# Jiahao-Ma/VFA

Hardware: AMD Instinct MI355X
Metric: voxels aggregated/sec (7 views->BEV grid) (higher is better)
Workload: dtype f32; 1 GPU; multiviewc_200x200x1; cameras_per_rank=7, cameras_total=7, channels=256, rccl_ranks=1, parallelism=single GPU

## Files before the change

include/vfa_hip.h:

```cpp
#ifndef VFA_HIP_H
#define VFA_HIP_H

#include <stddef.h>
#include <stdint.h>

#ifdef __cplusplus
extern "C" {
#endif

#define VFA_ABI_VERSION 9

#define VFA_CONV_MULTIVIEWC 0
#define VFA_CONV_MULTIVIEWX 1
#define VFA_CONV_WILDTRACK 2

#define VFA_VOX_REFERENCE 0
#define VFA_VOX_LAYER_MAJOR 1

#define VFA_VOX_KERNEL_DIRECT 0x100
#define VFA_VOX_KERNEL_TAP_CACHE 0x200

#define VFA_ERR_BAD_ARGUMENT 10001
#define VFA_ERR_UNSUPPORTED 10002

int vfa_abi_version(void);

#define VFA_FLAG_TERMS_MASK 0xf
#define VFA_FLAG_RESERVED_CUS(n) (((n) & 0xff) << 8)
#define VFA_FLAG_DEBUG(mask) (((mask) & 0xfff) << 16)
#define VFA_FLAG_DUMP_VOX (1 << 30)
#define VFA_FLAG_ROWS_ONLY (1 << 28)
#define VFA_FLAG_SKIP_ROWS (1 << 29)
#define VFA_BWD_ACCUMULATE 1

int vfa_integral_image_f32(const float *feature, float *integral, int n_views, int C, int Hf, int Wf,
                           void *stream);

int vfa_affine_relu_integral_image_f32(const float *x, const float *scale, const float *shift, float *integral, int n_views, int C,
                                       int Hf, int Wf, void *stream);

size_t vfa_feature_stats_count(int n_views, int C, int Hf);
int vfa_integral_images_f32(const float *const *features, const float *const *scales, const float *const *shifts,
                            float *const *integrals, unsigned *const *absmax, int n_views, int C, int n_maps, const int *feat_hw,
                            void *stream);
int vfa_integral_absmax_f32(const float *integral, unsigned *absmax, int n_views, int C, int Hf, int Wf, void *stream);

int vfa_integral_images_hwc_f32(const float *const *features_hwc, const float *const *scales, const float *const *shifts,
                                float *const *integrals, unsigned *const *absmax, int n_views, int C, int n_maps, const int *feat_hw,
                                void *stream);

size_t vfa_lateral_conv_workspace_bytes(int n_views, int Hf, int Wf);
int vfa_lateral_conv_f32(const float *feat, const float *weight, const float *bias, const float *gamma, const float *beta, float eps,
                         float *out_hwc, float *scale, float *shift, void *workspace, size_t workspace_bytes, int n_views, int K,
                         int Hf, int Wf, void *stream);
int vfa_lateral_convs_f32(int n_maps, const float *const *feats, const float *const *weights, const float *const *biases,
                          const float *const *gammas, const float *const *betas, const float *eps, float *const *outs_hwc,
                          float *const *scales, float *const *shifts, void *const *workspaces, const size_t *workspace_bytes, int n_views,
                          const int *Ks, const int *feat_hw, void *stream);

int vfa_lateral_convs_train_f32(int n_maps, const float *const *feats, const float *const *weights, const float *const *biases,
                                const float *const *gammas, const float *const *betas, const float *eps, float *const *outs_hwc,
                                float *const *scales, float *const *shifts, double *const *means, double *const *rstds,
// ... 210 lines not shown
```

vfa_amd/_lib.py:

```python
import ctypes
import os

_HERE = os.path.dirname(os.path.abspath(__file__))
LIB_PATH = os.environ.get("VFA_AMD_LIB") or os.path.join(_HERE, "csrc", "libvfa_hip.so")
ABI_VERSION = 9

CONV_KIND = {"MultiviewC": 0, "MultiviewX": 1, "Wildtrack": 2}
VOX_REFERENCE, VOX_LAYER_MAJOR = 0, 1
VOX_KERNEL_DIRECT, VOX_KERNEL_TAP_CACHE = 0x100, 0x200
BWD_ACCUMULATE = 1


FLAG_ROWS_ONLY, FLAG_SKIP_ROWS = 1 << 28, 1 << 29
FLAG_DUMP_VOX = 1 << 30


def collapse_flags(terms=0, reserved_cus=0):
    return (int(terms) & 0xf) | ((int(reserved_cus) & 0xff) << 8)


_c_int, _c_float, _c_size_t, _vp, _c_longlong = ctypes.c_int, ctypes.c_float, ctypes.c_size_t, ctypes.c_void_p, ctypes.c_longlong
_c_double = ctypes.c_double

SIGNATURES = {
    "vfa_abi_version": [],
    "vfa_integral_image_f32": [_vp, _vp, _c_int, _c_int, _c_int, _c_int, _vp],
    "vfa_affine_relu_integral_image_f32": [_vp, _vp, _vp, _vp, _c_int, _c_int, _c_int, _c_int, _vp],
    "vfa_box_params_f32": [_vp, _vp, _vp, _vp, _c_int, _c_int, _c_int, _c_int, _c_float, _c_float, _c_int, _c_int,
                           _c_float, _c_float, _vp, _vp, _vp, _vp],
    "vfa_gather_f32": [_vp, _vp, _vp, _vp, _vp, _c_int, _c_int, _c_int, _c_int, _c_int, _c_int, _c_int, _c_int, _c_int,
                       _vp],
    "vfa_project_gather_f32": [_vp, _vp, _vp, _vp, _vp, _vp, _c_int, _c_int, _c_int, _c_int, _c_int, _c_int, _c_int,
                               _c_int, _c_int, _c_float, _c_float, _c_float, _c_float, _c_int, _vp],
    "vfa_project_collapse_f32": [_vp, _vp, _vp, _vp, _vp, _vp, _vp, _c_int, _c_int, _c_int, _c_int, _c_int, _c_int, _c_int,
                                 _c_int, _c_float, _c_float, _c_float, _c_float, _vp],
    "vfa_gather_workspace_bytes": [_c_int, _c_int, _c_int],
    "vfa_project_gather_ws_f32": [_vp, _vp, _vp, _vp, _vp, _vp, _vp, _c_size_t, _c_int, _c_int, _c_int, _c_int, _c_int,
                                  _c_int, _c_int, _c_int, _c_int, _c_float, _c_float, _c_float, _c_float, _c_int, _vp],
    "vfa_project_gather_backward_f32": [_vp, _vp, _vp, _vp, _vp, _vp, _c_int, _c_int, _c_int, _c_int, _c_int, _c_int,
                                        _c_int, _c_int, _c_int, _c_float, _c_float, _c_float, _c_float, _c_int, _vp],
    "vfa_project_gather_backward_grid_f32": [_vp, _vp, _vp, _vp, _vp, _vp, _c_int, _c_int, _c_int, _c_int, _c_int, _c_int,
                                             _c_int, _c_int, _c_int, _c_int, _c_float, _c_float, _c_float, _c_float, _c_int, _vp],
    "vfa_gather_backward_det_workspace_bytes": [_c_int, _c_int, _c_int, _c_int, _c_int, _c_int],
    "vfa_project_gather_backward_det_f32": [_vp, _vp, _vp, _vp, _vp, _vp, _c_int, _c_int, _c_int, _c_int, _c_int, _c_int,
                                            _c_int, _c_int, _c_int, _c_int, _c_float, _c_float, _c_float, _c_float, _c_int, _vp,
                                            _c_size_t, _vp],
    "vfa_gather_backward_geometry_workspace_bytes": [_c_int, _c_int],
# ... 150 lines not shown
```

vfa_amd/csrc/vfa_fused.hip:

```cpp
#include <hip/hip_runtime.h>
#include <stdint.h>
#include <type_traits>

#include "vfa_geom.h"
#include "vfa_split.h"
#include "vfa_tile.h"

#ifndef VFA_TICKET_ORDER
#define VFA_TICKET_ORDER __ATOMIC_RELAXED
#endif

namespace {
using namespace vfa_dev;

constexpr int kRecBytes = 96;
constexpr int kMaxSlots = 123;
constexpr unsigned kItemCost = 704, kRowItemCost = 522;
constexpr int kRecSlots = 3;
constexpr int kThreads = 512;
constexpr int kRowBytes = 2 * kC;
constexpr int kPlane = kTileBoxes * kRowBytes;
constexpr int kSteps = kC / 16;

constexpr int kCont = 1 << 8;
constexpr int kTileRows = 4;
constexpr int kTileShiftAt = 8;

typedef int i32x8 __attribute__((ext_vector_type(8)));

struct RecordArgs {
    BoxGeom g;
    int n_views, L, W, tiles_w, n_tiles, n_scales;
    ScaleDims dims[kMaxScales];
    unsigned *live[kMaxScales];
    unsigned *direct[kMaxScales];
    unsigned *overflow[kMaxScales];
    unsigned *row_counter;
    unsigned rows_cap;
    unsigned *row_list;
    unsigned char *hdrs[kMaxScales];
    unsigned char *recs[kMaxScales];
    unsigned short *item_w;
    int views_pad;
};

__global__ __launch_bounds__(kWave) void frame_records_kernel(RecordArgs a)
{
    __shared__ uint4 stage[2][kTileBoxes * 6];
    const TileLane ln = tile_lane(a.n_views, a.n_tiles, a.tiles_w, a.L, a.W);
    const int lane = threadIdx.x, half = ln.half, b = ln.b, view = ln.view, tile = ln.tile;
    const bool pair_ok = ln.pair_ok, valid = ln.valid;

    float l, t, r, bt;
    cube_box(a.g, a.g.calibs + (size_t)view * 12, ln.cell, 0, l, t, r, bt);
#pragma unroll 1
    for (int s = 0; s < a.n_scales; ++s) {
        const int Hf = a.dims[s].Hf, Wf = a.dims[s].Wf;
        const float area = box_area(l, t, r, bt, Hf, Wf);
        const bool vis = valid && box_visible(area, Hf, Wf);
        const float masked = valid ? area * 0.0f : 0.0f;
        const bool live_box = vis || (valid && masked != masked);
        const BoxTaps tp = box_taps(l, t, r, bt, Hf, Wf);
        const int dx = tp.xr.i0 - tp.xl.i0, dy = tp.yb.i0 - tp.yt.i0;
        const int dxc = dx == 0 ? 0 : (dx == 1 ? 1 : 2), dyc = dy == 0 ? 0 : (dy == 1 ? 1 : 2);
        const TileWindow tw = tile_window(tp, vis, live_box, area, Hf, Wf, half);
        const Window &win = tw.w;
        const bool any_live = tw.any_live;
        const int shift = tw.shift, n_slots = win.n_slots;
        const bool direct = n_slots > kMaxSlots;
        unsigned rows[4], cols[4];
        tap_parts(win, tp, direct, rows, cols);
        const int tag = (vis ? 1 : 0) | (dxc << 1) | (dyc << 3);
        const unsigned kx = (unsigned)(tp.xs[0] + 1) | ((unsigned)(tp.xs[2] + 1) << 16), ky = (unsigned)(tp.ys[0] + 1) | ((unsigned)(tp.ys[2] + 1) << 16);
        const int tag_p = __shfl_up(tag, 1);
        const unsigned kx_p = __shfl_up(kx, 1), ky_p = __shfl_up(ky, 1);
        const bool cont = vis && (b & 3) != 0 && tag_p == tag && kx_p == kx && ky_p == ky;
// ... 6 lines not shown
            bilinear_weights(q, tp.xr, tp.yt); w[8] = q[0]; w[9] = q[1]; w[10] = q[2]; w[11] = q[3];
            bilinear_weights(q, tp.xl, tp.yb); w[12] = q[0]; w[13] = q[1]; w[14] = q[2]; w[15] = q[3];
        }
        if (pair_ok) {
            uint4 *st = stage[half] + b * 6;
            st[0] = make_uint4(__float_as_uint(w[0]), __float_as_uint(w[1]), __float_as_uint(w[2]), __float_as_uint(w[3]));
            st[1] = make_uint4(__float_as_uint(w[4]), __float_as_uint(w[5]), __float_as_uint(w[6]), __float_as_uint(w[7]));
            st[2] = make_uint4(__float_as_uint(w[8]), __float_as_uint(w[9]), __float_as_uint(w[10]), __float_as_uint(w[11]));
            st[3] = make_uint4(__float_as_uint(w[12]), __float_as_uint(w[13]), __float_as_uint(w[14]), __float_as_uint(w[15]));
            const float rcp = 1.0f / area;
            st[4] = make_uint4(__float_as_uint(rcp), (unsigned)tag | (cont ? (unsigned)kCont : 0u), rows[0] | (rows[1] << 16),
                               rows[2] | (rows[3] << 16));
            st[5] = make_uint4(cols[0] | (cols[1] << 16), cols[2] | (cols[3] << 16), __float_as_uint(masked), __float_as_uint(area));
        }
        __syncthreads();
        if (pair_ok) {
            uint4 *rec = reinterpret_cast<uint4 *>(a.recs[s] + ((size_t)view * a.n_tiles + tile) * kTileBoxes * kRecBytes);
#pragma unroll
            for (int k = 0; k < 6; ++k) rec[k * 32 + b] = stage[half][k * 32 + b];
            if (b == 0) {
                uint4 *hdr = reinterpret_cast<uint4 *>(a.hdrs[s] + ((size_t)view * a.n_tiles + tile) * kHdrBytes);
                unsigned hflags = (any_live ? kTileLive : 0) | (direct ? kTileDirect : 0) | ((unsigned)shift << kTileShiftAt), word2 = (unsigned)win.cwid;
                if (any_live) atomicOr(a.live[s] + tile, 1u << view);
                if (any_live && direct) {
                    atomicOr(a.direct[s] + tile, 1u << view);
                    const unsigned slot = atomicAdd(a.row_counter, 1u);
                    if (slot < a.rows_cap) {
                        hflags |= kTileRows; word2 = slot;
                        a.row_list[slot] = ((unsigned)s << 30) | ((unsigned)view << 25) | (unsigned)tile;
                    }
                    else atomicOr(a.overflow[s] + tile, 1u << view);
                }
                const bool main_item = any_live && !(direct && !(hflags & kTileRows));
                a.item_w[((size_t)tile * kMaxScales + s) * a.views_pad + view] =
                    (unsigned short)(!main_item ? 0u : (direct ? kRowItemCost : kItemCost + (unsigned)n_slots));
                hdr[0] = tile_header0(hflags, win, word2);
                hdr[1] = tile_header1(win);
            }
        }
        __syncthreads();
        if (blockIdx.x == 0 && lane < 6)
            reinterpret_cast<uint4 *>(a.recs[s] + (size_t)a.n_views * a.n_tiles * kTileBoxes * kRecBytes)[lane] = make_uint4(0u, 0u, 0u, 0u);
    }
}

struct ShiftArgs {
    BoxGeom g;
    int n_views, L, W, tiles_w, n_tiles, nl, Hf, Wf, per_item;
    unsigned char *out;
    unsigned *tile_max;
};
__global__ __launch_bounds__(kWave) void sliver_shift_kernel(ShiftArgs a)
{
    const TileLane ln = tile_lane(a.n_views, a.n_tiles, a.tiles_w, a.L, a.W);
    const float *P = a.g.calibs + (size_t)ln.view * 12;
    int shift = 0;
    for (int layer = 0; layer < a.nl; ++layer) {
        float l, t, r, bt;
        cube_box(a.g, P, ln.cell, layer, l, t, r, bt);
        const float area = box_area(l, t, r, bt, a.Hf, a.Wf);
        if (ln.valid && box_visible(area, a.Hf, a.Wf)) shift = max(shift, sliver_shift(area, a.Hf, a.Wf));
    }
#pragma unroll
    for (int m = 1; m < 32; m <<= 1) shift = max(shift, __shfl_xor(shift, m, 32));
    if (a.per_item) {
        if (ln.valid) a.out[(size_t)ln.view * a.L * a.W + ln.cell] = (unsigned char)shift;
    } else if (ln.pair_ok && ln.b == 0 && shift > 0) {
        atomicMax(a.tile_max + ln.tile, (unsigned)shift);
    }
}
__global__ __launch_bounds__(256) void sliver_expand_kernel(const unsigned *tile_max, unsigned char *out, int L, int W, int tiles_w)
{
    const int cell = blockIdx.x * 256 + threadIdx.x;
    if (cell >= L * W) return;
    const int cl = cell / W, cw = cell - cl * W;
    out[cell] = (unsigned char)tile_max[(cl / kTileL) * tiles_w + cw / kTileW];
}

constexpr int kWmaxParts = 32;
struct SplitArgs { const float *w[kMaxScales]; uint4 *out[kMaxScales]; unsigned *wmax; int *wexp; int f16; };
constexpr int kSplitBlocks = 8 * kSteps * 64 / 1024;
__device__ __forceinline__ void split_block(const SplitArgs &sa, int b, unsigned long long *part)
{
    const int scale = b / kSplitBlocks, j = b - scale * kSplitBlocks, tid = threadIdx.x;
    const float *__restrict__ w = sa.w[scale];
    uint4 *__restrict__ out = sa.out[scale];
    int ew = 0;
    if (sa.f16) {
        unsigned m = 0u;
        for (int i = tid; i < kC * kC; i += 1024) m = max(m, __float_as_uint(w[i]) & 0x7fffffffu);
        m = wave_max_u32(m);
        if ((tid & 63) == 0) part[tid >> 6] = m;
        __syncthreads();
        unsigned mm = 0u;
        for (int i = 0; i < 16; ++i) mm = max(mm, (unsigned)part[i]);
        ew = split_exponent(mm, kExpW);
    }
    const int idx = j * 1024 + tid;
    const int lane = idx & 63, st = (idx >> 6) & 15, wave = idx >> 10;
    const float *src = w + (size_t)(wave * 32 + (lane & 31)) * kC + 16 * st + 8 * (lane >> 5);
    if (idx == 0 && scale == 0) sa.wexp[kMaxScales] = sa.f16 ? 2 : 3;
    uint4 uh, ul;
    if (sa.f16) {
        fp16_saturate_mode(true);
        if (idx == 0) sa.wexp[scale] = ew;
        const float sc = pow2f(ew);
        uint2 h0, l0, h1, l1;
        split_f16x4(src[0] * sc, src[1] * sc, src[2] * sc, src[3] * sc, h0, l0);
        split_f16x4(src[4] * sc, src[5] * sc, src[6] * sc, src[7] * sc, h1, l1);
        uh = make_uint4(h0.x, h0.y, h1.x, h1.y);
        ul = make_uint4(l0.x, l0.y, l1.x, l1.y);
    } else {
        union { __bf16 b[8]; uint4 u; } hi, lo;
#pragma unroll
        for (int k = 0; k < 8; ++k) {
            const float x = src[k];
            hi.b[k] = (__bf16)x;
            lo.b[k] = (__bf16)(x - (float)hi.b[k]);
        }
        uh = hi.u; ul = lo.u;
    }
    out[((size_t)(wave * kSteps + st) * 2 + 0) * 64 + lane] = uh;
    out[((size_t)(wave * kSteps + st) * 2 + 1) * 64 + lane] = ul;
}

struct ChunkArgs {
    const unsigned *live[kMaxScales], *overflow[kMaxScales];
    const unsigned short *item_w;
    int n_scales, n_tiles, n_views, views_pad;
    int *chunk_start, *chunk_rank;
    SplitArgs split;
    int n_split_blocks;
};
template <int G> struct TileItemsT { unsigned m[kMaxScales]; uint4 q[kMaxScales][G]; };
template <int G>
__global__ __launch_bounds__(1024) void tile_chunks_kernel(ChunkArgs a)
{
    using TileItems = TileItemsT<G>;
    constexpr bool kCache = G == 1;
    __shared__ unsigned long long part[1024];
    if (blockIdx.x > 0) {
        split_block(a.split, (int)blockIdx.x - 1, part);
        return;
    }
    const int tid = threadIdx.x, n_tiles = a.n_tiles;
    const unsigned view_mask = a.n_views >= 32 ? 0xffffffffu : ((1u << a.n_views) - 1u);
    const int per = (n_tiles + 1023) / 1024, t0 = min(n_tiles, tid * per), t1 = min(n_tiles, t0 + per);
    constexpr unsigned kScale = 294, kTile = 330, kEmpty = 32;
    struct RawTile { unsigned lv[kMaxScales], ov[kMaxScales]; uint4 q[kMaxScales][G]; };
    auto load_raw = [&](int t) {
        RawTile rt;
#pragma unroll
        for (int s = 0; s < kMaxScales; ++s) {
            const bool on = s < a.n_scales;
            const unsigned *lp = on ? a.live[s] : a.live[0], *op = on ? a.overflow[s] : a.overflow[0];
            rt.lv[s] = lp[t]; rt.ov[s] = op[t];
#pragma unroll
            for (int g = 0; g < G; ++g) {
                const int gg = g * 8 < a.n_views ? g : 0;
                rt.q[s][g] = *reinterpret_cast<const uint4 *>(a.item_w + ((size_t)t * kMaxScales + (on ? s : 0)) * a.views_pad + 8 * gg);
            }
        }
        return rt;
    };
    auto finish_tile = [&](const RawTile &rt) {
        TileItems ti;
#pragma unroll
        for (int s = 0; s < kMaxScales; ++s) {
            const bool on = s < a.n_scales;
            ti.m[s] = on ? rt.lv[s] & ~rt.ov[s] & view_mask : 0u;
#pragma unroll
            for (int g = 0; g < G; ++g) ti.q[s][g] = (!on || g * 8 >= a.n_views) ? make_uint4(0u, 0u, 0u, 0u) : rt.q[s][g];
        }
        return ti;
    };
    auto load_tile = [&](int t) { return finish_tile(load_raw(t)); };
    auto walk = [&](const TileItems &ti, auto &&visit) -> unsigned {
        unsigned w = 0;
        int k = 0;
#pragma unroll
        for (int s = 0; s < kMaxScales; ++s) {
// ... 31 lines not shown
    part[tid] = local;
    for (int c = tid; c <= kChunks; c += 1024) { a.chunk_start[c] = n_tiles; a.chunk_rank[c] = 0; }
    __syncthreads();
    for (int d = 1; d < 1024; d <<= 1) {
        const unsigned long long v = tid >= d ? part[tid - d] : 0ull;
        __syncthreads();
        part[tid] += v;
        __syncthreads();
    }
    const unsigned long long total = part[1023];
    unsigned long long before = part[tid] - local;
    auto pos_of = [&](long long cc) { return (total * (unsigned long long)cc + kChunks - 1) / kChunks; };
    for (int t = t0; t < t1; ++t) {
        const unsigned long long tb = before;
        long long c = tb > 0 ? (long long)((tb - 1) * kChunks / total) : 0;
        while (c < kChunks && pos_of(c) < tb) ++c;
        const TileItems ti = tile_of(t);
        int n_items = 0;
        walk(ti, [&](int kk, unsigned, unsigned) { n_items = kk + 1; });
        const unsigned w = walk(ti, [&](int kk, unsigned w0, unsigned w1) {
            while (c < kChunks) {
                const unsigned long long pc = pos_of(c);
                if (pc >= tb + w1) break;
                const int k = ((unsigned)(pc - tb) - w0) * 2 < (w1 - w0) ? kk : kk + 1;
                if (k >= n_items) { a.chunk_start[c] = t + 1 < n_tiles ? t + 1 : n_tiles; a.chunk_rank[c] = 0; }
                else { a.chunk_start[c] = t; a.chunk_rank[c] = k; }
                ++c;
            }
        });
        if (n_items == 0)
            for (; c < kChunks && pos_of(c) < tb + w; ++c) { a.chunk_start[c] = t; a.chunk_rank[c] = 0; }
        before += w;
    }
}

struct FusedScale {
    const float *integral;
    const float *bias;
    const uint4 *wfrag;
    const unsigned *live, *direct, *overflow;
    const unsigned char *hdrs, *recs;
    int Hf, Wf;
    const unsigned *amax;
    int amax_n;
};
struct FusedArgs {
    FusedScale sc[kMaxScales];
    int n_scales, n_views, L, W, tiles_w, n_tiles;
    float *out;
    const int *chunk_start, *chunk_rank;
    float *partial;
    unsigned *tickets;
    const float *rows;
    const unsigned *row_counter;
    int rows_cap;
    int accumulate;
    const int *wexp;
    int debug;
    unsigned long long *diag;
};
constexpr int kDbgNoFills = 1, kDbgNoPool = 2, kDbgNoMfma = 4, kDbgOneW = 8, kDbgNoRecords = 16, kDbgNoExtra = 32, kDbgStamps = 128;
constexpr int kDbgDumpVox = 0x1000;

struct LRec { uint4 v[6]; };

template <bool F16>
// ... 783 lines not shown
        const uint4 *rp = reinterpret_cast<const uint4 *>(a.recs[s] + ((size_t)item * kTileBoxes + b) * kRecBytes);
        uint4 r[6];
#pragma unroll
        for (int k = 0; k < 6; ++k) r[k] = rp[k];
        const float wt[16] = {__uint_as_float(r[0].x), __uint_as_float(r[0].y), __uint_as_float(r[0].z), __uint_as_float(r[0].w),
                              __uint_as_float(r[1].x), __uint_as_float(r[1].y), __uint_as_float(r[1].z), __uint_as_float(r[1].w),
                              __uint_as_float(r[2].x), __uint_as_float(r[2].y), __uint_as_float(r[2].z), __uint_as_float(r[2].w),
                              __uint_as_float(r[3].x), __uint_as_float(r[3].y), __uint_as_float(r[3].z), __uint_as_float(r[3].w)};
        const float rcp = __uint_as_float(r[4].x), masked = __uint_as_float(r[5].z), area = __uint_as_float(r[5].w);
        const bool vis = (r[4].y & (unsigned)kVis) != 0u;
        const unsigned rws[4] = {vis ? r[4].z & 0xffffu : 0u, vis ? r[4].z >> 16 : 0u, vis ? r[4].w & 0xffffu : 0u, vis ? r[4].w >> 16 : 0u};
        const unsigned cls[4] = {vis ? r[5].x & 0xffffu : 0u, vis ? r[5].x >> 16 : 0u, vis ? r[5].y & 0xffffu : 0u, vis ? r[5].y >> 16 : 0u};
        const char *img = reinterpret_cast<const char *>(a.integral[s]) + (size_t)view * (a.Hf[s] + 2) * Wp * kSlotBytes + q * 256 + cq * 16;
        float4 t[4][4];
#pragma unroll
        for (int i = 0; i < 4; ++i)
#pragma unroll
            for (int j = 0; j < 4; ++j) t[i][j] = *reinterpret_cast<const float4 *>(img + (size_t)(rws[i] * Wp + cls[j]) * kSlotBytes);
        __builtin_amdgcn_sched_barrier(0);
        const float4 lt = sample4(t[0][0], t[0][1], t[1][0], t[1][1], wt[0], wt[1], wt[2], wt[3]);
        const float4 rb = sample4(t[2][2], t[2][3], t[3][2], t[3][3], wt[4], wt[5], wt[6], wt[7]);
        const float4 rt = sample4(t[0][2], t[0][3], t[1][2], t[1][3], wt[8], wt[9], wt[10], wt[11]);
        const float4 lb2 = sample4(t[2][0], t[2][1], t[3][0], t[3][1], wt[12], wt[13], wt[14], wt[15]);
        float4 res = make_float4(box_mean(lt.x, rb.x, rt.x, lb2.x, area, rcp), box_mean(lt.y, rb.y, rt.y, lb2.y, area, rcp),
                                 box_mean(lt.z, rb.z, rt.z, lb2.z, area, rcp), box_mean(lt.w, rb.w, rt.w, lb2.w, area, rcp));
        if (!vis) res = make_float4(masked, masked, masked, masked);
        reinterpret_cast<float4 *>(a.rows)[((size_t)slot * kTileBoxes + b) * (kC / 4) + q * 16 + cq] = res;
    }
}


struct WorkspaceLayout {
    size_t live[kMaxScales], direct[kMaxScales], overflow[kMaxScales], counter, hdrs[kMaxScales], recs[kMaxScales], wfrag[kMaxScales],
        masks_bytes, chunks, ranks, diag, rows, row_list, partial, tickets, item_w, wmax, wexp, amax, total;
    int tiles_l, tiles_w, n_tiles, rows_cap, views_pad;
};
inline WorkspaceLayout layout_of(int n_views, int L, int W, int n_scales)
{
    WorkspaceLayout w;
    w.tiles_l = (L + kTileL - 1) / kTileL;
    w.tiles_w = (W + kTileW - 1) / kTileW;
    w.n_tiles = w.tiles_l * w.tiles_w;
    size_t off = 0;
    for (int s = 0; s < kMaxScales; ++s) {
        const bool on = s < n_scales;
        w.live[s] = off;  off = align_up(off + (on ? (size_t)w.n_tiles * 4 : 0), 256);
        w.direct[s] = off; off = align_up(off + (on ? (size_t)w.n_tiles * 4 : 0), 256);
        w.overflow[s] = off; off = align_up(off + (on ? (size_t)w.n_tiles * 4 : 0), 256);
    }
    w.counter = off; off += 256;
    w.tickets = off; off = align_up(off + (size_t)w.n_tiles * sizeof(unsigned), 256);
    w.masks_bytes = off;
    for (int s = 0; s < kMaxScales; ++s) {
        const bool on = s < n_scales;
        w.hdrs[s] = off;  off = align_up(off + (on ? (size_t)n_views * w.n_tiles * kHdrBytes : 0), 256);
        w.recs[s] = off;  off = align_up(off + (on ? ((size_t)n_views * w.n_tiles * kTileBoxes + 1) * kRecBytes : 0), 256);
        w.wfrag[s] = off; off = align_up(off + (on ? (size_t)8 * kSteps * 2 * 64 * 16 : 0), 256);
    }
    w.chunks = off;
    off = align_up(off + (kChunks + 1) * sizeof(int), 256);
    w.ranks = off;
    off = align_up(off + (kChunks + 1) * sizeof(int), 256);
    w.partial = off;
    off = align_up(off + (size_t)kMaxBlocks * 2 * 8 * 16 * 64 * sizeof(float), 256);
    w.diag = off;
    off = align_up(off + 512 * 8 * sizeof(unsigned long long), 256);
    const size_t items = (size_t)n_views * w.n_tiles * n_scales;
    size_t cap = items / 4 + 64;
    if (cap > 8192) cap = 8192;
    if (items * (size_t)(kTileBoxes * kC * sizeof(float)) <= ((size_t)1 << 30)) cap = items;
    if (cap > items) cap = items;
    w.rows_cap = (int)cap;
    w.row_list = off;
    off = align_up(off + cap * sizeof(unsigned), 256);
    w.wmax = off; off = align_up(off + (size_t)kMaxScales * kWmaxParts * sizeof(unsigned), 256);
    w.wexp = off; off = align_up(off + (kMaxScales + 1) * sizeof(int), 256);
    w.amax = off; off = align_up(off + (size_t)kMaxScales * kFallbackStats * sizeof(unsigned), 256);
    w.views_pad = (n_views + 7) / 8 * 8;
    w.item_w = off;
    off = align_up(off + (size_t)w.n_tiles * kMaxScales * w.views_pad * sizeof(unsigned short) + 16, 256);
    w.rows = off;
    off = align_up(off + cap * kTileBoxes * kC * sizeof(float), 256);
    w.total = off;
    return w;
}

inline int rows_cap_of(const WorkspaceLayout &lay, size_t bytes)
{
    if (bytes <= lay.rows) return 0;
    const size_t fit = (bytes - lay.rows) / ((size_t)kTileBoxes * kC * sizeof(float));
    return fit < (size_t)lay.rows_cap ? (int)fit : lay.rows_cap;
}

}

extern "C" {

size_t vfa_frame_workspace_bytes(int n_views, int L, int W, int n_scales)
{
    if (n_views < 0 || L < 0 || W < 0 || n_scales < 1 || n_scales > kMaxScales) return 0;
    return layout_of(n_views, L, W, n_scales).total;
}

int vfa_frame_workspace_layout(int n_views, int L, int W, int n_scales, size_t *offsets, int *tiles)
{
    if (n_views < 0 || L < 0 || W < 0 || n_scales < 1 || n_scales > kMaxScales || !offsets || !tiles) return VFA_ERR_BAD_ARGUMENT;
    const WorkspaceLayout lay = layout_of(n_views, L, W, n_scales);
// ... 14 lines not shown
    offsets[24] = lay.ranks;
    tiles[0] = lay.tiles_l;
    tiles[1] = lay.tiles_w;
    tiles[2] = kMaxSlots;
    tiles[3] = kChunks;
    return 0;
}

int vfa_frame_boxes_f32(const float *calibs, const float *grid, const float *z_layers, const float *corner_off, int n_views, int L,
                        int W, int conv_kind, float img_w, float img_h, float cmin, float cmax, int n_scales,
                        const int *feat_hw, void *workspace, size_t workspace_bytes, void *stream)
{
    if (n_views < 0 || L < 0 || W < 0 || n_scales < 1 || n_scales > kMaxScales || conv_kind < 0 || conv_kind > 2 || !feat_hw)
        return VFA_ERR_BAD_ARGUMENT;
    if (n_views > 32) return VFA_ERR_UNSUPPORTED;
    const WorkspaceLayout lay = layout_of(n_views, L, W, n_scales);
    if (lay.n_tiles == 0 || n_views == 0) return 0;
    if ((long long)n_views * lay.n_tiles >= (1ll << 31) - 2 || lay.n_tiles >= (1 << 25)) return VFA_ERR_UNSUPPORTED;
    if (!workspace || workspace_bytes < lay.rows) return VFA_ERR_BAD_ARGUMENT;
    hipStream_t s = (hipStream_t)stream;
    unsigned char *ws = reinterpret_cast<unsigned char *>(workspace);
    RecordArgs a;
    a.g = BoxGeom{calibs, grid, z_layers, corner_off, conv_kind, img_w, img_h, cmin, cmax};
    a.n_views = n_views; a.L = L; a.W = W; a.tiles_w = lay.tiles_w; a.n_tiles = lay.n_tiles; a.n_scales = n_scales;
    for (int k = 0; k < kMaxScales; ++k) {
        a.dims[k].Hf = k < n_scales ? feat_hw[2 * k] : 1;
        a.dims[k].Wf = k < n_scales ? feat_hw[2 * k + 1] : 1;
        if (a.dims[k].Hf <= 0 || a.dims[k].Wf <= 0 || a.dims[k].Hf > 65533 || a.dims[k].Wf > 65533) return VFA_ERR_BAD_ARGUMENT;
        a.live[k] = reinterpret_cast<unsigned *>(ws + lay.live[k]);
        a.direct[k] = reinterpret_cast<unsigned *>(ws + lay.direct[k]);
        a.overflow[k] = reinterpret_cast<unsigned *>(ws + lay.overflow[k]);
        a.hdrs[k] = ws + lay.hdrs[k];
        a.recs[k] = ws + lay.recs[k];
    }
    a.row_counter = reinterpret_cast<unsigned *>(ws + lay.counter);
    a.rows_cap = (unsigned)rows_cap_of(lay, workspace_bytes);
    a.row_list = reinterpret_cast<unsigned *>(ws + lay.row_list);
    a.item_w = reinterpret_cast<unsigned short *>(ws + lay.item_w);
    a.views_pad = lay.views_pad;
    const hipError_t e = zero_fill(ws, lay.masks_bytes, s);
    if (e != hipSuccess) return (int)e;
    const long long pairs = (long long)n_views * lay.n_tiles;
    hipLaunchKernelGGL(frame_records_kernel, dim3((unsigned)((pairs + 1) / 2)), dim3(kWave), 0, s, a);
    return (int)hipGetLastError();
}

int vfa_frame_cuts_f32(int n_views, int L, int W, int n_scales, const float *const *weights, int flags, void *workspace,
                       size_t workspace_bytes, void *stream)
{
    const int terms = flags & VFA_FLAG_TERMS_MASK;
    if ((flags & ~VFA_FLAG_TERMS_MASK) || (terms != 0 && terms != 2 && terms != 3 && terms != 4)) return VFA_ERR_BAD_ARGUMENT;
    if (n_views < 0 || L < 0 || W < 0 || n_scales < 1 || n_scales > kMaxScales) return VFA_ERR_BAD_ARGUMENT;
    if (n_views > 32) return VFA_ERR_UNSUPPORTED;
    const WorkspaceLayout lay = layout_of(n_views, L, W, n_scales);
    if (lay.n_tiles == 0 || n_views == 0) return 0;
    if (!workspace || workspace_bytes < lay.rows) return VFA_ERR_BAD_ARGUMENT;
    hipStream_t s = (hipStream_t)stream;
    unsigned char *ws = reinterpret_cast<unsigned char *>(workspace);
    ChunkArgs ca;
    for (int k = 0; k < kMaxScales; ++k) {
        const int q = k < n_scales ? k : 0;
        ca.live[k] = reinterpret_cast<const unsigned *>(ws + lay.live[q]);
        ca.overflow[k] = reinterpret_cast<const unsigned *>(ws + lay.overflow[q]);
    }
    ca.n_scales = n_scales; ca.n_tiles = lay.n_tiles; ca.n_views = n_views; ca.views_pad = lay.views_pad;
    ca.item_w = reinterpret_cast<const unsigned short *>(ws + lay.item_w);
    ca.chunk_start = reinterpret_cast<int *>(ws + lay.chunks);
    ca.chunk_rank = reinterpret_cast<int *>(ws + lay.ranks);
    ca.split = SplitArgs{};
    ca.n_split_blocks = 0;
    if (weights) {
        SplitArgs &sa = ca.split;
        for (int k = 0; k < kMaxScales; ++k) {
            sa.w[k] = weights[k < n_scales ? k : 0];
            sa.out[k] = reinterpret_cast<uint4 *>(ws + lay.wfrag[k < n_scales ? k : 0]);
            if (!sa.w[k]) return VFA_ERR_BAD_ARGUMENT;
        }
        sa.wmax = reinterpret_cast<unsigned *>(ws + lay.wmax);
        sa.wexp = reinterpret_cast<int *>(ws + lay.wexp);
        sa.f16 = (terms == 0 || terms == 2) ? 1 : 0;
        ca.n_split_blocks = n_scales * kSplitBlocks;
    }
    if (n_views <= 8) hipLaunchKernelGGL(tile_chunks_kernel<1>, dim3(1 + ca.n_split_blocks), dim3(1024), 0, s, ca);
    else hipLaunchKernelGGL(tile_chunks_kernel<4>, dim3(1 + ca.n_split_blocks), dim3(1024), 0, s, ca);
    return (int)hipGetLastError();
}

int vfa_frame_records_f32(const float *calibs, const float *grid, const float *z_layers, const float *corner_off, int n_views, int L,
                          int W, int conv_kind, float img_w, float img_h, float cmin, float cmax, int n_scales,
                          const int *feat_hw, const float *const *weights, int flags, void *workspace, size_t workspace_bytes, void *stream)
{
    const int st = vfa_frame_boxes_f32(calibs, grid, z_layers, corner_off, n_views, L, W, conv_kind, img_w, img_h, cmin, cmax, n_scales, feat_hw,
                                       workspace, workspace_bytes, stream);
    if (st) return st;
    return vfa_frame_cuts_f32(n_views, L, W, n_scales, weights, flags, workspace, workspace_bytes, stream);
}

int vfa_pool_windows_f32(const float *integral, const void *workspace, size_t workspace_bytes, float *vox, int n_views, int L, int W,
                         int n_scales, int scale, int Hf, int Wf, void *stream)
{
    if (n_views < 0 || L < 0 || W < 0 || n_scales < 1 || n_scales > kMaxScales || scale < 0 || scale >= n_scales || Hf <= 0 || Wf <= 0)
        return VFA_ERR_BAD_ARGUMENT;
    if (n_views > 32) return VFA_ERR_UNSUPPORTED;
    const WorkspaceLayout lay = layout_of(n_views, L, W, n_scales);
    if (lay.n_tiles == 0 || n_views == 0) return 0;
    if (!workspace || workspace_bytes < lay.rows || !integral || !vox) return VFA_ERR_BAD_ARGUMENT;
    const unsigned char *ws = reinterpret_cast<const unsigned char *>(workspace);
    PoolArgs a;
    a.integral = integral; a.hdrs = ws + lay.hdrs[scale]; a.recs = ws + lay.recs[scale]; a.vox = vox;
    a.direct = reinterpret_cast<const unsigned *>(ws + lay.direct[scale]);
    a.n_views = n_views; a.L = L; a.W = W; a.tiles_w = lay.tiles_w; a.n_tiles = lay.n_tiles; a.Hf = Hf; a.Wf = Wf;
    const long long units = (long long)n_views * lay.n_tiles * 4;
    if (units >= (1ll << 31) - 8) return VFA_ERR_UNSUPPORTED;
    a.per_xcd = 0;
    int n_cu = 256;
    {
        int dev = 0, cus = 0;
// ... 166 lines not shown
```

vfa_amd/ops.py:

```python
import os
import ctypes

import torch

from . import _lib


def _f32c(t):
    return t.to(dtype=torch.float32).contiguous()


class KernelTimer:
    active = None

    def __init__(self, only=None, every=1):
        self.records = []
        self.only = None if only is None else frozenset(only)
        self.every = max(int(every), 1)
        self.seen = {}

    def __enter__(self):
        KernelTimer.active = self
        return self

# ... 667 lines not shown
        assert absmax.dtype == torch.int32 and absmax.is_contiguous()
        rows = tiles = None
        if shift is not None:
            assert shift.dtype == torch.uint8 and shift.shape[-1] == cells and shift.numel() in (cells, n * cells)
            rows = shift.reshape(-1, cells).expand(n, cells).contiguous().view(-1)
            pad = (-rows.numel()) % 128
            tiles = (torch.nn.functional.pad(rows, (0, pad)) if pad else rows).view(-1, 128).amax(dim=1).contiguous()
        _launch("vfa_collapse_gemm_relu_backward_f16_f32", _lib.ptr(vox), _lib.ptr(weight), _lib.ptr(bias) if bias is not None else None,
                _lib.ptr(grad_out), _lib.ptr(glin), _lib.ptr(gbias), _lib.ptr(ws), ws.numel(), n, cells, K, 256, _lib.ptr(absmax),
                absmax.numel(), _lib.ptr(rows) if rows is not None else None, _lib.ptr(tiles) if tiles is not None else None,
                _lib.collapse_flags(0, reserved_cus), _lib.current_stream_handle(), tag=(n, cells, K, "f16"))
    else:
        _launch("vfa_collapse_gemm_relu_backward_f32", _lib.ptr(vox), _lib.ptr(weight), _lib.ptr(bias) if bias is not None else None,
                _lib.ptr(grad_out), _lib.ptr(glin), _lib.ptr(gbias), _lib.ptr(ws), ws.numel(), n, cells, K, 256,
                _lib.collapse_flags(terms, reserved_cus), _lib.current_stream_handle(), tag=(n, cells, K))
    if det:
        gbias = column_sum(glin.view(n * cells, 256))
    return glin, gbias


def sliver_shifts(calibs, grid, z_layers, corner_off, conv_kind, image_wh, feat_hw, per_item, crange=(-1, 0.95)):
    calibs, grid, z_layers, corner_off = _geometry(calibs, grid, z_layers, corner_off)
    n, (L, W) = calibs.shape[0], grid.shape[:2]
    out = torch.empty((n if per_item else 1, L * W), dtype=torch.uint8, device=calibs.device)
    need = _lib.lib().vfa_sliver_shifts_scratch_bytes(L, W)
    scratch = torch.empty(max(need, 16), dtype=torch.uint8, device=calibs.device)
    _launch("vfa_sliver_shifts_u8", _lib.ptr(calibs), _lib.ptr(grid), _lib.ptr(z_layers), z_layers.numel(), _lib.ptr(corner_off), n, L, W,
            int(conv_kind), float(image_wh[0]), float(image_wh[1]), float(crange[0]), float(crange[1]), int(feat_hw[0]), int(feat_hw[1]),
            1 if per_item else 0, _lib.ptr(out), _lib.ptr(scratch), scratch.numel(), _lib.current_stream_handle(), tag=(n, L, W))
    return out


def frame_records(calibs, grid, z_layers, corner_off, conv_kind, image_wh, feat_hws, weights=None, crange=(-1, 0.95),
                  workspace=None, row_slots=None, cuts=True, terms=0):
    calibs, grid, z_layers, corner_off = _geometry(calibs, grid, z_layers, corner_off)
    n, (L, W) = calibs.shape[0], grid.shape[:2]
    if z_layers.numel() != 1:
        raise _lib.VFAHipError("frame_records / pool_collapse cover single-layer grids (nl = 1) only")
    ns = len(feat_hws)
    need = _lib.lib().vfa_frame_workspace_bytes(n, L, W, ns)
    if row_slots is not None:
        lay = frame_workspace_layout(n, L, W, ns)
        need = lay["rows"] + min(int(row_slots), lay["rows_cap"]) * 32 * 256 * 4
        workspace = None
    if workspace is None or workspace.numel() < need:
        workspace = torch.empty(max(need, 1), dtype=torch.uint8, device=calibs.device)
    hw = _lib.int_array([v for f in feat_hws for v in f])
    wts = _weight_ptrs(weights, ns, (256, 256))
    if not cuts:
        _launch("vfa_frame_boxes_f32", _lib.ptr(calibs), _lib.ptr(grid), _lib.ptr(z_layers), _lib.ptr(corner_off), n, L, W,
                int(conv_kind), float(image_wh[0]), float(image_wh[1]), float(crange[0]), float(crange[1]), ns, hw,
                _lib.ptr(workspace), workspace.numel(), _lib.current_stream_handle(), tag=(n, L, W, ns))
        return workspace
    _launch("vfa_frame_records_f32", _lib.ptr(calibs), _lib.ptr(grid), _lib.ptr(z_layers), _lib.ptr(corner_off), n, L, W,
            int(conv_kind), float(image_wh[0]), float(image_wh[1]), float(crange[0]), float(crange[1]), ns, hw, wts, int(terms) & 0xf,
            _lib.ptr(workspace), workspace.numel(), _lib.current_stream_handle(), tag=(n, L, W, ns))
    return workspace


def frame_cuts(workspace, n_views, grid_lw, n_scales, weights=None, terms=0):
    _lib.require_device(workspace)
    wts = _weight_ptrs(weights, n_scales, (256, 256))
    _launch("vfa_frame_cuts_f32", int(n_views), int(grid_lw[0]), int(grid_lw[1]), int(n_scales), wts, int(terms) & 0xf, _lib.ptr(workspace),
            workspace.numel(), _lib.current_stream_handle(), tag=(int(n_views), int(grid_lw[0]), int(grid_lw[1]), int(n_scales)))
    return workspace


def pool_collapse(integrals, biases, workspace, grid_lw, out=None, accumulate=False, terms=0, reserved_cus=0, debug=0, stage="all",
                  absmax=None, dump_vox=False):
    _lib.require_device(*integrals, workspace, out)
    stage_flag = {"all": 0, "rows": _lib.FLAG_ROWS_ONLY, "main": _lib.FLAG_SKIP_ROWS}[stage]
    ns = len(integrals)
    n = integrals[0].shape[0]
    L, W = grid_lw
    assert all(i.shape[0] == n and i.shape[3] == 256 and i.is_contiguous() and i.dtype == torch.float32 for i in integrals)
    if out is None and stage != "rows":
        out = torch.empty((L * W, 256), dtype=torch.float32, device=integrals[0].device)
        accumulate = False
    assert out is None or (out.dtype == torch.float32 and out.is_contiguous() and tuple(out.shape) == (L * W, 256)), \
        "out must be a contiguous fp32 (L*W, 256) tensor"
    biases = [None if b is None else _f32c(b) for b in (biases if biases is not None else [None] * ns)]
    hw = _lib.int_array([v for i in integrals for v in (i.shape[1] - 2, i.shape[2] - 2)])
    absmax, absmax_ptrs = _absmax_of(integrals, absmax)
    _launch("vfa_pool_collapse_relu_sum_f32", _lib.ptr_array(list(integrals)), absmax_ptrs, _lib.ptr_array(biases), _lib.ptr(workspace),
            workspace.numel(), _lib.ptr(out) if out is not None else None, n, L, W, ns, hw, 1 if accumulate else 0,
            _lib.collapse_flags(terms, reserved_cus) | ((int(debug) & 0xfff) << 16) | stage_flag | (_lib.FLAG_DUMP_VOX if dump_vox else 0),
            _lib.current_stream_handle(), tag=(n, L, W, tuple((i.shape[1] - 2, i.shape[2] - 2) for i in integrals), stage))
    return out


def pool_windows(integral, workspace, grid_lw, n_scales, scale, out=None):
    _lib.require_device(integral, workspace, out)
    n, Hp, Wp, C = integral.shape
    assert C == 256 and integral.is_contiguous() and integral.dtype == torch.float32
    L, W = grid_lw
    vox = out if out is not None else torch.empty((n, L * W, 256), dtype=torch.float32, device=integral.device)
# ... 308 lines not shown
```

Measured before the change: 1.550 billion voxels/s.

## Compute chunk cuts with parallel prefix scan and per-thread binary search

Replaces the single-block serial walk that assigns work chunks to tiles with a multi-block kernel. Each block computes per-tile weights from per-tile cost sums accumulated atomically in the records kernel, does a shared-memory prefix scan, and each thread binary-searches its own cut position. The weight-split blocks also move to a 512-thread variant with vectorized absmax loads. The old walk stays available behind a flag. This adds atomics in the records kernel, extra workspace, and redundant per-block scans in exchange for removing a serial bottleneck in a small setup kernel.

After: 1.550 billion voxels/s (median of 2 runs). Within noise of the previous version (+0.0%).

```diff
diff --git a/include/vfa_hip.h b/include/vfa_hip.h
--- a/include/vfa_hip.h
+++ b/include/vfa_hip.h
@@ -28,6 +28,7 @@
 #define VFA_FLAG_TERMS_MASK 0xf
 #define VFA_FLAG_RESERVED_CUS(n) (((n) & 0xff) << 8)
 #define VFA_FLAG_DEBUG(mask) (((mask) & 0xfff) << 16)
+#define VFA_FLAG_CUTS_WALK (1 << 16)
 #define VFA_FLAG_DUMP_VOX (1 << 30)
 #define VFA_FLAG_ROWS_ONLY (1 << 28)
 #define VFA_FLAG_SKIP_ROWS (1 << 29)
diff --git a/vfa_amd/_lib.py b/vfa_amd/_lib.py
--- a/vfa_amd/_lib.py
+++ b/vfa_amd/_lib.py
@@ -13,6 +13,7 @@
 
 FLAG_ROWS_ONLY, FLAG_SKIP_ROWS = 1 << 28, 1 << 29
 FLAG_DUMP_VOX = 1 << 30
+FLAG_CUTS_WALK = 1 << 16
 
 
 def collapse_flags(terms=0, reserved_cus=0):
diff --git a/vfa_amd/csrc/vfa_cuts.h b/vfa_amd/csrc/vfa_cuts.h
--- /dev/null
+++ b/vfa_amd/csrc/vfa_cuts.h
@@ -0,0 +1,96 @@
+#ifndef VFA_CUTS_H
+#define VFA_CUTS_H
+
+#if defined(__HIPCC__)
+#define VFA_CUTS_HD __host__ __device__ __forceinline__
+#define VFA_CUTS_UNROLL _Pragma("unroll")
+#else
+#define VFA_CUTS_HD inline
+#define VFA_CUTS_UNROLL
+#endif
+
+namespace vfa_cuts {
+
+constexpr int kCutScales = 3;
+constexpr unsigned kScale = 294, kTile = 330, kEmpty = 32;
+
+struct Cut { int start, rank; };
+
+VFA_CUTS_HD unsigned tile_weight(int n_scales, const unsigned *m, const unsigned *sum)
+{
+    unsigned w = 0;
+    bool any = false;
+    VFA_CUTS_UNROLL
+    for (int s = 0; s < kCutScales; ++s)
+        if (s < n_scales && m[s]) { w += sum[s] + kScale; any = true; }
+    return any ? w + kTile : kEmpty;
+}
+
+VFA_CUTS_HD unsigned long long cut_position(unsigned long long total, long long c, int n_chunks)
+{
+    return (total * (unsigned long long)c + (unsigned long long)(n_chunks - 1)) / (unsigned long long)n_chunks;
+}
+
+template <class Before>
+VFA_CUTS_HD int find_interval(int n, unsigned long long p, Before &&before)
+{
+    int lo = 0, hi = n;
+    while (hi - lo > 1) {
+        const int mid = lo + (hi - lo) / 2;
+        if (before(mid) <= p) lo = mid;
+        else hi = mid;
+    }
+    return lo;
+}
+
+template <class Cost>
+VFA_CUTS_HD Cut cut_in_tile(int t, int n_tiles, int n_scales, const unsigned *m, Cost &&cost, unsigned off)
+{
+    const Cut next = {t + 1 < n_tiles ? t + 1 : n_tiles, 0};
+    int n_items = 0;
+    VFA_CUTS_UNROLL
+    for (int s = 0; s < kCutScales; ++s)
+        if (s < n_scales) n_items += __builtin_popcount(m[s]);
+    Cut cut = {t, 0};
+    if (n_items == 0) return cut;
+    cut = next;
+    unsigned w = 0;
+    int k = 0;
+    bool found = false;
+    VFA_CUTS_UNROLL
+    for (int s = 0; s < kCutScales; ++s) {
+        unsigned ms = s < n_scales ? m[s] : 0u;
+        bool first = true;
+        while (ms && !found) {
+            const int v = __builtin_ctz(ms);
+            ms &= ms - 1u;
+            const unsigned wi = cost(s, v) + (first ? kScale : 0u) + (k == 0 ? kTile : 0u);
+            first = false;
+            if (off < w + wi) {
+                const int kk = (off - w) * 2u < wi ? k : k + 1;
+                if (kk < n_items) { cut.start = t; cut.rank = kk; }
+                found = true;
+            }
+            w += wi;
+            ++k;
+        }
+    }
+    return cut;
+}
+
+template <class Before, class Masks, class Cost>
+VFA_CUTS_HD Cut cut_of_chunk(long long c, int n_chunks, unsigned long long total, int n_tiles, int n_scales, Before &&before, Masks &&masks,
+                             Cost &&cost)
+{
+    const unsigned long long p = cut_position(total, c, n_chunks);
+    if (p >= total) { const Cut end = {n_tiles, 0}; return end; }
+    const int t = find_interval(n_tiles, p, before);
+    unsigned m[kCutScales];
+    VFA_CUTS_UNROLL
+    for (int s = 0; s < kCutScales; ++s) m[s] = s < n_scales ? masks(t, s) : 0u;
+    return cut_in_tile(t, n_tiles, n_scales, m, [&](int s, int v) { return cost(t, s, v); }, (unsigned)(p - before(t)));
+}
+
+}
+
+#endif
diff --git a/vfa_amd/csrc/vfa_fused.hip b/vfa_amd/csrc/vfa_fused.hip
--- a/vfa_amd/csrc/vfa_fused.hip
+++ b/vfa_amd/csrc/vfa_fused.hip
@@ -5,6 +5,7 @@
 #include "vfa_geom.h"
 #include "vfa_split.h"
 #include "vfa_tile.h"
+#include "vfa_cuts.h"
 
 #ifndef VFA_TICKET_ORDER
 #define VFA_TICKET_ORDER __ATOMIC_RELAXED
@@ -42,6 +43,7 @@
     unsigned char *recs[kMaxScales];
     unsigned short *item_w;
     int views_pad;
+    unsigned *cost_sum[kMaxScales];
 };
 
 __global__ __launch_bounds__(kWave) void frame_records_kernel(RecordArgs a)
@@ -114,8 +116,9 @@
                     else atomicOr(a.overflow[s] + tile, 1u << view);
                 }
                 const bool main_item = any_live && !(direct && !(hflags & kTileRows));
-                a.item_w[((size_t)tile * kMaxScales + s) * a.views_pad + view] =
-                    (unsigned short)(!main_item ? 0u : (direct ? kRowItemCost : kItemCost + (unsigned)n_slots));
+                const unsigned cost = !main_item ? 0u : (direct ? kRowItemCost : kItemCost + (unsigned)n_slots);
+                a.item_w[((size_t)tile * kMaxScales + s) * a.views_pad + view] = (unsigned short)cost;
+                if (main_item) atomicAdd(a.cost_sum[s] + tile, cost);
                 hdr[0] = tile_header0(hflags, win, word2);
                 hdr[1] = tile_header1(win);
             }
@@ -161,24 +164,34 @@
 
 constexpr int kWmaxParts = 32;
 struct SplitArgs { const float *w[kMaxScales]; uint4 *out[kMaxScales]; unsigned *wmax; int *wexp; int f16; };
-constexpr int kSplitBlocks = 8 * kSteps * 64 / 1024;
+template <int T>
 __device__ __forceinline__ void split_block(const SplitArgs &sa, int b, unsigned long long *part)
 {
+    constexpr int kSplitBlocks = 8 * kSteps * 64 / T;
     const int scale = b / kSplitBlocks, j = b - scale * kSplitBlocks, tid = threadIdx.x;
     const float *__restrict__ w = sa.w[scale];
     uint4 *__restrict__ out = sa.out[scale];
     int ew = 0;
     if (sa.f16) {
         unsigned m = 0u;
-        for (int i = tid; i < kC * kC; i += 1024) m = max(m, __float_as_uint(w[i]) & 0x7fffffffu);
+        if ((reinterpret_cast<uintptr_t>(w) & 15u) == 0) {
+            const uint4 *__restrict__ w4 = reinterpret_cast<const uint4 *>(w);
+#pragma unroll 8
+            for (int i = tid; i < kC * kC / 4; i += T) {
+                const uint4 x = w4[i];
+                m = max(max(m, x.x & 0x7fffffffu), max(max(x.y & 0x7fffffffu, x.z & 0x7fffffffu), x.w & 0x7fffffffu));
+            }
+        } else {
+            for (int i = tid; i < kC * kC; i += T) m = max(m, __float_as_uint(w[i]) & 0x7fffffffu);
+        }
         m = wave_max_u32(m);
         if ((tid & 63) == 0) part[tid >> 6] = m;
         __syncthreads();
         unsigned mm = 0u;
-        for (int i = 0; i < 16; ++i) mm = max(mm, (unsigned)part[i]);
+        for (int i = 0; i < T / 64; ++i) mm = max(mm, (unsigned)part[i]);
         ew = split_exponent(mm, kExpW);
     }
-    const int idx = j * 1024 + tid;
+    const int idx = j * T + tid;
     const int lane = idx & 63, st = (idx >> 6) & 15, wave = idx >> 10;
     const float *src = w + (size_t)(wave * 32 + (lane & 31)) * kC + 16 * st + 8 * (lane >> 5);
     if (idx == 0 && scale == 0) sa.wexp[kMaxScales] = sa.f16 ? 2 : 3;
@@ -213,6 +226,8 @@
     int *chunk_start, *chunk_rank;
     SplitArgs split;
     int n_split_blocks;
+    const unsigned *cost_sum[kMaxScales];
+    unsigned *tile_w;
 };
 template <int G> struct TileItemsT { unsigned m[kMaxScales]; uint4 q[kMaxScales][G]; };
 template <int G>
@@ -222,13 +237,13 @@
     constexpr bool kCache = G == 1;
     __shared__ unsigned long long part[1024];
     if (blockIdx.x > 0) {
-        split_block(a.split, (int)blockIdx.x - 1, part);
+        split_block<1024>(a.split, (int)blockIdx.x - 1, part);
         return;
     }
     const int tid = threadIdx.x, n_tiles = a.n_tiles;
     const unsigned view_mask = a.n_views >= 32 ? 0xffffffffu : ((1u << a.n_views) - 1u);
     const int per = (n_tiles + 1023) / 1024, t0 = min(n_tiles, tid * per), t1 = min(n_tiles, t0 + per);
-    constexpr unsigned kScale = 294, kTile = 330, kEmpty = 32;
+    using vfa_cuts::kScale; using vfa_cuts::kTile; using vfa_cuts::kEmpty;
     struct RawTile { unsigned lv[kMaxScales], ov[kMaxScales]; uint4 q[kMaxScales][G]; };
     auto load_raw = [&](int t) {
         RawTile rt;
@@ -326,6 +341,112 @@
             for (; c < kChunks && pos_of(c) < tb + w; ++c) { a.chunk_start[c] = t; a.chunk_rank[c] = 0; }
         before += w;
     }
+}
+
+constexpr int kCutThreads = 512, kCutBlocks = kChunks / kCutThreads, kCutLds = 4096;
+static_assert(kCutBlocks * kCutThreads == kChunks, "one cut per thread");
+template <int G>
+__global__ __launch_bounds__(kCutThreads) void tile_cuts_kernel(ChunkArgs a)
+{
+    constexpr int T = kCutThreads, kPer = 4;
+    __shared__ unsigned long long s_before[kCutLds];
+    __shared__ unsigned long long part[T];
+    if (blockIdx.x >= kCutBlocks) {
+        split_block<T>(a.split, (int)blockIdx.x - kCutBlocks, part);
+        return;
+    }
+    const int tid = threadIdx.x, n_tiles = a.n_tiles, n_scales = a.n_scales;
+    const unsigned view_mask = a.n_views >= 32 ? 0xffffffffu : ((1u << a.n_views) - 1u);
+    const int g = (n_tiles + kCutLds - 1) / kCutLds, n_gran = (n_tiles + g - 1) / g;
+    for (int i = tid; i < n_gran; i += T) s_before[i] = 0ull;
+    __syncthreads();
+    auto load_masks = [&](int t, unsigned (&lv)[kMaxScales], unsigned (&ov)[kMaxScales]) {
+#pragma unroll
+        for (int s = 0; s < kMaxScales; ++s) { const int q = s < n_scales ? s : 0; lv[s] = a.live[q][t]; ov[s] = a.overflow[q][t]; }
+    };
+    auto masks_of = [&](const unsigned (&lv)[kMaxScales], const unsigned (&ov)[kMaxScales], unsigned (&m)[kMaxScales]) {
+#pragma unroll
+        for (int s = 0; s < kMaxScales; ++s) m[s] = s < n_scales ? lv[s] & ~ov[s] & view_mask : 0u;
+    };
+    for (int base = 0; base < n_tiles; base += kPer * T) {
+        unsigned lv[kPer][kMaxScales], ov[kPer][kMaxScales], sm[kPer][kMaxScales];
+#pragma unroll
+        for (int j = 0; j < kPer; ++j) {
+            const int t = min(base + j * T + tid, n_tiles - 1);
+            load_masks(t, lv[j], ov[j]);
+#pragma unroll
+            for (int s = 0; s < kMaxScales; ++s) sm[j][s] = a.cost_sum[s < n_scales ? s : 0][t];
+        }
+        __builtin_amdgcn_sched_barrier(0);
+#pragma unroll
+        for (int j = 0; j < kPer; ++j) {
+            const int t = base + j * T + tid;
+            unsigned m[kMaxScales];
+            masks_of(lv[j], ov[j], m);
+            const unsigned w = vfa_cuts::tile_weight(n_scales, m, sm[j]);
+            if (t < n_tiles) {
+                if (g > 1) a.tile_w[t] = w;
+                atomicAdd(&s_before[t / g], (unsigned long long)w);
+            }
+        }
+    }
+    __syncthreads();
+    const int per = (n_gran + T - 1) / T, g0 = min(n_gran, tid * per), g1 = min(n_gran, g0 + per);
+    unsigned long long local = 0;
+    for (int i = g0; i < g1; ++i) local += s_before[i];
+    part[tid] = local;
+    __syncthreads();
+    for (int d = 1; d < T; d <<= 1) {
+        const unsigned long long v = tid >= d ? part[tid - d] : 0ull;
+        __syncthreads();
+        part[tid] += v;
+        __syncthreads();
+    }
+    const unsigned long long total = part[T - 1];
+    {
+        unsigned long long run = part[tid] - local;
+        for (int i = g0; i < g1; ++i) { const unsigned long long w = s_before[i]; s_before[i] = run; run += w; }
+    }
+    __syncthreads();
+
+    const int c = (int)blockIdx.x * T + tid;
+    if (c == 0) { a.chunk_start[kChunks] = n_tiles; a.chunk_rank[kChunks] = 0; }
+    const unsigned long long p = vfa_cuts::cut_position(total, c, kChunks);
+    const int gi = vfa_cuts::find_interval(n_gran, p, [&](int i) { return s_before[i]; });
+    int t = gi * g;
+    unsigned long long before = s_before[gi];
+    if (g > 1) {
+        unsigned long long acc = before;
+        for (int j = 0; j < g; ++j) {
+            const int tt = min(gi * g + j, n_tiles - 1);
+            const unsigned w = a.tile_w[tt];
+            if (gi * g + j < n_tiles && p >= acc) { t = tt; before = acc; }
+            acc += w;
+        }
+    }
+    unsigned lv[kMaxScales], ov[kMaxScales], m[kMaxScales];
+    uint4 q[kMaxScales][G];
+    load_masks(t, lv, ov);
+#pragma unroll
+    for (int s = 0; s < kMaxScales; ++s)
+#pragma unroll
+        for (int gg = 0; gg < G; ++gg)
+            q[s][gg] = *reinterpret_cast<const uint4 *>(a.item_w + ((size_t)t * kMaxScales + (s < n_scales ? s : 0)) * a.views_pad +
+                                                        8 * (gg * 8 < a.n_views ? gg : 0));
+    masks_of(lv, ov, m);
+    auto cost = [&](int s, int v) {
+        uint4 x = q[0][0];
+#pragma unroll
+        for (int s2 = 0; s2 < kMaxScales; ++s2)
+#pragma unroll
+            for (int gg = 0; gg < G; ++gg)
+                if (s == s2 && (v >> 3) == gg) x = q[s2][gg];
+        const unsigned pair = (v & 4) ? ((v & 2) ? x.w : x.z) : ((v & 2) ? x.y : x.x);
+        return (pair >> (16 * (v & 1))) & 0xffffu;
+    };
+    const vfa_cuts::Cut cut = vfa_cuts::cut_in_tile(t, n_tiles, n_scales, m, cost, (unsigned)(p - before));
+    a.chunk_start[c] = cut.start;
+    a.chunk_rank[c] = cut.rank;
 }
 
 struct FusedScale {
@@ -1175,7 +1296,7 @@
 
 struct WorkspaceLayout {
     size_t live[kMaxScales], direct[kMaxScales], overflow[kMaxScales], counter, hdrs[kMaxScales], recs[kMaxScales], wfrag[kMaxScales],
-        masks_bytes, chunks, ranks, diag, rows, row_list, partial, tickets, item_w, wmax, wexp, amax, total;
+        masks_bytes, chunks, ranks, diag, rows, row_list, partial, tickets, item_w, wmax, wexp, amax, cost_sum[kMaxScales], tile_w, total;
     int tiles_l, tiles_w, n_tiles, rows_cap, views_pad;
 };
 inline WorkspaceLayout layout_of(int n_views, int L, int W, int n_scales)
@@ -1193,6 +1314,9 @@
     }
     w.counter = off; off += 256;
     w.tickets = off; off = align_up(off + (size_t)w.n_tiles * sizeof(unsigned), 256);
+    for (int s = 0; s < kMaxScales; ++s) {
+        w.cost_sum[s] = off; off = align_up(off + (s < n_scales ? (size_t)w.n_tiles * sizeof(unsigned) : 0), 256);
+    }
     w.masks_bytes = off;
     for (int s = 0; s < kMaxScales; ++s) {
         const bool on = s < n_scales;
@@ -1216,6 +1340,8 @@
     w.rows_cap = (int)cap;
     w.row_list = off;
     off = align_up(off + cap * sizeof(unsigned), 256);
+    w.tile_w = off;
+    off = align_up(off + (size_t)w.n_tiles * sizeof(unsigned), 256);
     w.wmax = off; off = align_up(off + (size_t)kMaxScales * kWmaxParts * sizeof(unsigned), 256);
     w.wexp = off; off = align_up(off + (kMaxScales + 1) * sizeof(int), 256);
     w.amax = off; off = align_up(off + (size_t)kMaxScales * kFallbackStats * sizeof(unsigned), 256);
@@ -1296,6 +1422,7 @@
         a.overflow[k] = reinterpret_cast<unsigned *>(ws + lay.overflow[k]);
         a.hdrs[k] = ws + lay.hdrs[k];
         a.recs[k] = ws + lay.recs[k];
+        a.cost_sum[k] = reinterpret_cast<unsigned *>(ws + lay.cost_sum[k]);
     }
     a.row_counter = reinterpret_cast<unsigned *>(ws + lay.counter);
     a.rows_cap = (unsigned)rows_cap_of(lay, workspace_bytes);
@@ -1313,7 +1440,8 @@
                        size_t workspace_bytes, void *stream)
 {
     const int terms = flags & VFA_FLAG_TERMS_MASK;
-    if ((flags & ~VFA_FLAG_TERMS_MASK) || (terms != 0 && terms != 2 && terms != 3 && terms != 4)) return VFA_ERR_BAD_ARGUMENT;
+    const bool walk = (flags & VFA_FLAG_CUTS_WALK) != 0;
+    if ((flags & ~(VFA_FLAG_TERMS_MASK | VFA_FLAG_CUTS_WALK)) || (terms != 0 && terms != 2 && terms != 3 && terms != 4)) return VFA_ERR_BAD_ARGUMENT;
     if (n_views < 0 || L < 0 || W < 0 || n_scales < 1 || n_scales > kMaxScales) return VFA_ERR_BAD_ARGUMENT;
     if (n_views > 32) return VFA_ERR_UNSUPPORTED;
     const WorkspaceLayout lay = layout_of(n_views, L, W, n_scales);
@@ -1326,7 +1454,9 @@
         const int q = k < n_scales ? k : 0;
         ca.live[k] = reinterpret_cast<const unsigned *>(ws + lay.live[q]);
         ca.overflow[k] = reinterpret_cast<const unsigned *>(ws + lay.overflow[q]);
-    }
+        ca.cost_sum[k] = reinterpret_cast<const unsigned *>(ws + lay.cost_sum[q]);
+    }
+    ca.tile_w = reinterpret_cast<unsigned *>(ws + lay.tile_w);
     ca.n_scales = n_scales; ca.n_tiles = lay.n_tiles; ca.n_views = n_views; ca.views_pad = lay.views_pad;
     ca.item_w = reinterpret_cast<const unsigned short *>(ws + lay.item_w);
     ca.chunk_start = reinterpret_cast<int *>(ws + lay.chunks);
@@ -1343,10 +1473,14 @@
         sa.wmax = reinterpret_cast<unsigned *>(ws + lay.wmax);
         sa.wexp = reinterpret_cast<int *>(ws + lay.wexp);
         sa.f16 = (terms == 0 || terms == 2) ? 1 : 0;
-        ca.n_split_blocks = n_scales * kSplitBlocks;
-    }
-    if (n_views <= 8) hipLaunchKernelGGL(tile_chunks_kernel<1>, dim3(1 + ca.n_split_blocks), dim3(1024), 0, s, ca);
-    else hipLaunchKernelGGL(tile_chunks_kernel<4>, dim3(1 + ca.n_split_blocks), dim3(1024), 0, s, ca);
+        ca.n_split_blocks = n_scales * (8 * kSteps * 64 / (walk ? 1024 : kCutThreads));
+    }
+    if (walk) {
+        if (n_views <= 8) hipLaunchKernelGGL(tile_chunks_kernel<1>, dim3(1 + ca.n_split_blocks), dim3(1024), 0, s, ca);
+        else hipLaunchKernelGGL(tile_chunks_kernel<4>, dim3(1 + ca.n_split_blocks), dim3(1024), 0, s, ca);
+    }
+    else if (n_views <= 8) hipLaunchKernelGGL(tile_cuts_kernel<1>, dim3(kCutBlocks + ca.n_split_blocks), dim3(kCutThreads), 0, s, ca);
+    else hipLaunchKernelGGL(tile_cuts_kernel<4>, dim3(kCutBlocks + ca.n_split_blocks), dim3(kCutThreads), 0, s, ca);
     return (int)hipGetLastError();
 }
 
diff --git a/vfa_amd/ops.py b/vfa_amd/ops.py
--- a/vfa_amd/ops.py
+++ b/vfa_amd/ops.py
@@ -723,7 +723,7 @@
 
 
 def frame_records(calibs, grid, z_layers, corner_off, conv_kind, image_wh, feat_hws, weights=None, crange=(-1, 0.95),
-                  workspace=None, row_slots=None, cuts=True, terms=0):
+                  workspace=None, row_slots=None, cuts=True, terms=0, walk_cuts=False):
     calibs, grid, z_layers, corner_off = _geometry(calibs, grid, z_layers, corner_off)
     n, (L, W) = calibs.shape[0], grid.shape[:2]
     if z_layers.numel() != 1:
@@ -744,15 +744,17 @@
                 _lib.ptr(workspace), workspace.numel(), _lib.current_stream_handle(), tag=(n, L, W, ns))
         return workspace
     _launch("vfa_frame_records_f32", _lib.ptr(calibs), _lib.ptr(grid), _lib.ptr(z_layers), _lib.ptr(corner_off), n, L, W,
-            int(conv_kind), float(image_wh[0]), float(image_wh[1]), float(crange[0]), float(crange[1]), ns, hw, wts, int(terms) & 0xf,
+            int(conv_kind), float(image_wh[0]), float(image_wh[1]), float(crange[0]), float(crange[1]), ns, hw, wts,
+            (int(terms) & 0xf) | (_lib.FLAG_CUTS_WALK if walk_cuts else 0),
             _lib.ptr(workspace), workspace.numel(), _lib.current_stream_handle(), tag=(n, L, W, ns))
     return workspace
 
 
-def frame_cuts(workspace, n_views, grid_lw, n_scales, weights=None, terms=0):
+def frame_cuts(workspace, n_views, grid_lw, n_scales, weights=None, terms=0, walk_cuts=False):
     _lib.require_device(workspace)
     wts = _weight_ptrs(weights, n_scales, (256, 256))
-    _launch("vfa_frame_cuts_f32", int(n_views), int(grid_lw[0]), int(grid_lw[1]), int(n_scales), wts, int(terms) & 0xf, _lib.ptr(workspace),
+    _launch("vfa_frame_cuts_f32", int(n_views), int(grid_lw[0]), int(grid_lw[1]), int(n_scales), wts,
+            (int(terms) & 0xf) | (_lib.FLAG_CUTS_WALK if walk_cuts else 0), _lib.ptr(workspace),
             workspace.numel(), _lib.current_stream_handle(), tag=(int(n_views), int(grid_lw[0]), int(grid_lw[1]), int(n_scales)))
     return workspace
 
```
